# Ledicia/Molecular-Dynamics-Simulation---Lennard-Jones-monoatomic-fluid

Hardware: AMD Instinct MI355X
Metric: md_steps_per_sec_n262144_fp64 (higher is better)
Workload: dtype f64

## Files before the change

molecular-dynamics-simulation---lennard-jones-monoatomic-fluid_amd/csrc/ljmd_common.cpp:

```cpp
#include "ljmd_common.h"
#include "ljmd_internal.h"

#include <algorithm>
#include <cstdio>
#include <cstring>
#include <limits>

namespace ljmdh {

using namespace ljmdk;

thread_local std::string g_last_error = "";

int failv(std::string *handle_err, int code, const char *fmt, va_list ap)
{
    char buf[512];
    vsnprintf(buf, sizeof buf, fmt, ap);
    g_last_error = buf;
    if (handle_err) *handle_err = buf;
    return code;
}

int check_sim_params(const char *who, int n, double box_length, double dt, double rc)
{
// ... 51 lines not shown
        if (v && *v) return std::atoi(v);
        return std::nullopt;
    };
    Knobs k;
    k.sort = flag("LJMD_SORT", k.sort);
    k.force_generic = flag("LJMD_FORCE_GENERIC", k.force_generic);
    k.force_collectives = flag("LJMD_FORCE_COLLECTIVES", k.force_collectives);
    k.fuse = flag("LJMD_FUSE", k.fuse);
    k.fuse_tail = flag("LJMD_FUSE_TAIL", k.fuse_tail);
    k.fuse_defer_record = flag("LJMD_FUSE_DEFER_RECORD", k.fuse_defer_record);
    k.xcd_remap = std::max(0, env_int("LJMD_N3_XCD_REMAP", k.xcd_remap));
    k.inject_failure_at_step = env_int("LJMD_INJECT_FAILURE_AT_STEP", k.inject_failure_at_step);
    k.exchange_alltoall = is("LJMD_FORCE_EXCHANGE", "alltoall");
    k.resort_every = opt_int("LJMD_RESORT_EVERY");
    k.kd_sort_cub = is("LJMD_KD_SORT", "cub");
    k.n3_row_tiles = env_int("LJMD_N3_ROW_TILES", k.n3_row_tiles);
    k.n3_wg_waves = env_int("LJMD_N3_WG_WAVES", k.n3_wg_waves);
    k.slab_budget_gb = std::max(1, env_int("LJMD_SLAB_BUDGET_GB", k.slab_budget_gb));
    k.n3_both_ties = flag("LJMD_N3_BOTH_TIES", k.n3_both_ties);
    k.n3_min_n = env_int("LJMD_N3_MIN_N", k.n3_min_n);
    k.n3 = flag("LJMD_N3", k.n3);
    k.n3_target_waves = opt_int("LJMD_N3_TARGET_WAVES");
    k.n3_clusters = flag("LJMD_N3_CLUSTERS", k.n3_clusters);
    k.n3_pertile = flag("LJMD_N3_PERTILE", k.n3_pertile);
    k.reduce_split = opt_int("LJMD_REDUCE_SPLIT");
    if (k.reduce_split) k.reduce_split = std::max(0, *k.reduce_split);
    k.walk_chunk = opt_int("LJMD_WALK_CHUNK");
    k.vanhove_chunk = opt_int("LJMD_VANHOVE_CHUNK");
    k.fp32_far_stream = flag("LJMD_FP32_FAR_STREAM", k.fp32_far_stream);
    k.fp32_vfar = flag("LJMD_FP32_VFAR", k.fp32_vfar);
    {
        const char *rs = std::getenv("LJMD_FP32_SPLIT");
        if (rs && *rs) k.fp32_split = std::max(0.0, std::atof(rs));
    }
    k.overlap_exchange = flag("LJMD_OVERLAP_EXCHANGE", k.overlap_exchange);
    k.migrate_blocks = is("LJMD_MIGRATE_DEAL", "blocks");
    {
        const char *xm = std::getenv("LJMD_MULTI_EXCHANGE");
        k.multi_exchange = xm ? xm : "";
    }
    k.multi_migrate_every = std::max(0, env_int("LJMD_MULTI_MIGRATE_EVERY", k.multi_migrate_every));
    k.multi_threads = flag("LJMD_MULTI_THREADS", k.multi_threads);
    k.batch_group_streams = !is("LJMD_BATCH_GROUP_STREAMS", "0");
    return k;
}

// ... 72 lines not shown
```

molecular-dynamics-simulation---lennard-jones-monoatomic-fluid_amd/csrc/ljmd_common.h:

```cpp
#ifndef LJMD_COMMON_H
#define LJMD_COMMON_H

#include "ljmd.h"

#include <hip/hip_runtime.h>

#include <cstdarg>
#include <cstddef>
#include <cstdint>
#include <cstdlib>
#include <optional>
#include <string>

namespace ljmdh {

extern thread_local std::string g_last_error;

constexpr double kPi = 3.1415926535897932384626433832795;

int failv(std::string *handle_err, int code, const char *fmt, va_list ap);

inline int fail(std::nullptr_t, int code, const char *fmt, ...)
{
    va_list ap;
// ... 58 lines not shown
void scalars_from_exact_sums(const uint64_t (&ordered)[5][3], double te, double td, double tdd, bool have_e, bool have_k,
                             double *epot, double *ekin, double *d_epot, double *dd_epot);

struct Knobs {
    bool sort = true;
    bool force_generic = false;
    bool force_collectives = false;
    bool fuse = true;
    bool fuse_tail = true;
    bool fuse_defer_record = true;
    int xcd_remap = 4;
    int inject_failure_at_step = -1;
    bool exchange_alltoall = false;
    std::optional<int> resort_every;
    bool kd_sort_cub = false;
    int n3_row_tiles = 0;
    int n3_wg_waves = 0;
    int slab_budget_gb = 64;
    bool n3_both_ties = true;
    int n3_min_n = 4096;
    bool n3 = true;
    std::optional<int> n3_target_waves;
    bool n3_clusters = true;
    bool n3_pertile = true;
    std::optional<int> reduce_split;
    std::optional<int> walk_chunk;
    std::optional<int> vanhove_chunk;
    bool fp32_far_stream = true;
    bool fp32_vfar = true;
    double fp32_split = 5.0;
    bool overlap_exchange = true;
    bool migrate_blocks = false;
    std::string multi_exchange;
    int multi_migrate_every = 2000;
    bool multi_threads = true;
    bool batch_group_streams = true;
};
Knobs read_knobs();

}
#endif
```

molecular-dynamics-simulation---lennard-jones-monoatomic-fluid_amd/csrc/ljmd_engine.cpp:

```cpp
#include "ljmd_engine.h"

namespace ljmdh {

bool fast_path_ok(const ljmd_t *h) { return h->plan.rc_allows_fast && h->positions_compact && !h->knobs.force_generic; }

double *wg_part_now(ljmd_t *h) { return h->d_wg_part + (h->plan.fuse_tail ? (size_t)h->fold_parity * h->wg_part_stride : 0); }

PairArgs pair_args(ljmd_t *h, bool fast)
{
    PairArgs a;
    a.pos = h->d_pos;
    a.slab = h->d_slab;
    a.wg_part = wg_part_now(h);
    a.mask = h->d_mask;
    a.bbox = h->d_bbox;
    a.inline_mask = (fast && h->plan.fuse_tail && !h->plan.use_n3) ? 1 : 0;
    a.rc2_skin = h->rc2 * (1.0 + 1e-10);
    a.n = h->n;
    a.S = h->plan.S;
    a.P = h->plan.P;
    a.G = h->G;
    a.rank = h->rank;
    a.TB = h->plan.TB;
    a.T = h->plan.T;
// ... 42 lines not shown
    a.slab_i = h->d_slab;
    a.slab_j = h->d_slab_j;
    a.flag_j = h->d_flag_j;
    a.wg_part = wg_part_now(h);
    a.S = h->plan.S;
    a.P = h->plan.P;
    a.G = h->G;
    a.rank = h->rank;
    a.TB = h->plan.TB;
    a.T = h->plan.T;
    a.W = h->plan.W;
    a.NG = h->plan.NG;
    a.NGo = h->plan.NGo;
    a.Dmax = h->plan.Dmax;
    a.CS = h->plan.CS;
    a.by_group = h->plan.j_by_group;
    a.dchunk = h->plan.dchunk;
    a.uchunk = h->plan.uchunk;
    a.by0 = 0;
    a.xcd_remap = 0;
    a.inline_class = (h->plan.fuse_tail && h->plan.rt <= 2 && h->plan.wg_waves == 1) ? 1 : 0;
    a.both_ties = h->plan.both_ties ? 1 : 0;
    a.rc2_skin = h->rc2 * (1.0 + 1e-10);
    a.energy = h->want_energy ? 1 : 0;
    a.RT = h->plan.rt;
    a.L = h->L;
    a.invL = h->invL;
    a.rc2 = h->rc2;
    return a;
}

IntegrateArgs integrate_args(ljmd_t *h)
{
    IntegrateArgs a;
    a.r = own_block(h);
    a.ru = h->d_ru;
    a.v = h->d_v;
    a.a = h->d_a;
    a.fsum = needs_force_exchange(h) ? h->d_frecv : h->d_fpart;
    a.bbox = nullptr;
    a.pos_tc = nullptr;
    a.RT = std::max(1, h->plan.rt);
    a.ticket = nullptr;
    a.ke_part = h->d_ke_part;
    a.rows = h->plan.P;
    a.P = h->plan.P;
    a.L = h->L;
// ... 485 lines not shown
```

molecular-dynamics-simulation---lennard-jones-monoatomic-fluid_amd/csrc/ljmd_engine.h:

```cpp
#ifndef LJMD_ENGINE_H
#define LJMD_ENGINE_H

#include "ljmd_common.h"

#include <rccl/rccl.h>

#include <algorithm>
#include <cmath>
#include <cstdio>
#include <cstring>
#include <limits>
#include <mutex>
#include <vector>

#include "ljmd_internal.h"
#include "ljmd_resident.h"
#include "ljmd_sort.h"

using namespace ljmdk;

namespace ljmdh {

constexpr unsigned kRingCap = 4096;
constexpr int kTargetWorkgroups = 2048;
constexpr int kXcdMinGroups = 256;
constexpr int kMixedMinN = 16384;
constexpr long kN3ItemsFor4 = 6000;
constexpr long kN3ItemsFor2 = 1000;
constexpr long kN3LargeItems = 131072;
constexpr int kN3MidTargetItems = 32768;
constexpr int kBothTiesMaxGroups = 128;
constexpr int kFuseTailMaxRowTiles = 2;
constexpr int kFuseTailMaxN = 20000;
constexpr int kReduceSplitMinN = 131072;
constexpr int kReduceSplitShare = 8;
constexpr int kMaxProfiledLaunches = 4096;
constexpr int kEventsPerLaunch = 9;

struct EventSet {
    hipEvent_t e[kEventsPerLaunch];
    bool has_pos_x = false, has_force_x = false;
};

struct LaunchPlan {
    int S = 0, P = 0;
    int TB = 0, T = 0, W = 0;
    bool rc_allows_fast = false;
    bool sort_enabled = true;
    int resort_every = 20;
    std::vector<int> kd_level_nseg;
    std::vector<size_t> kd_level_off;
    std::vector<int> kd_offsets;
    int kd_finish_from = 0;
    int nslab_g = 1, chunk_g = 0;
    int nslab_t = 1, chunk_t = 0;
    bool use_n3 = false;
    int wg_waves = 1;
    bool both_ties = false;
    int uchunk = 0;
    int CS = 0, CS2 = 0, j_by_group = 0;
    int NG = 0, NGo = 0, Dmax = 0, nslab_n = 1, dchunk = 0;
    int rt = kRowTiles;
    bool fuse_tail = false;
    int split_s1 = 0, split_j1 = 0;
    int nslab_max = 1, n_wg_max = 0;
    int n_ke = 0;
};

int plan_engine(const SimParams &sim, int n, int n_ranks, int precision_mode, const Knobs &k, LaunchPlan *out);

}

struct ljmd_multi;

using namespace ljmdh;

struct ljmd : ljmdh::SimParams {
    ljmd_multi *multi = nullptr;
    bool poisoned = false;
    int inject_failure_at = -1;
    int n = 0, rank = 0, G = 1, device = 0, mode = 0;
    ljmdh::Knobs knobs;
// ... 160 lines not shown
```

molecular-dynamics-simulation---lennard-jones-monoatomic-fluid_amd/csrc/ljmd_kernels.hip:

```cpp
#include <hip/hip_runtime.h>
#include <stdint.h>

#include "ljmd_internal.h"

namespace ljmdk {

__device__ __forceinline__ double wave_min(double v)
{
#pragma unroll
    for (int off = 32; off > 0; off >>= 1) v = fmin(v, __shfl_down(v, off, 64));
    return v;
}

__device__ __forceinline__ double wave_max(double v)
{
#pragma unroll
    for (int off = 32; off > 0; off >>= 1) v = fmax(v, __shfl_down(v, off, 64));
    return v;
}

__global__ __launch_bounds__(kBlock) void pair_rows_generic_kernel(PairArgs a)
{
    __shared__ double red[2 * kWavesPerBlock];
    const int row = blockIdx.x * kBlock + threadIdx.x;
// ... 152 lines not shown
}

__device__ __forceinline__ double straddle(double e, double half)
{
    return e - __builtin_copysign(half, e);
}

template <int NU>
__device__ __forceinline__ void pair_disp(double xi, double yi, double zi, double xj, double yj, double zj, double L,
                                          double invL, double sx, double sy, double sz, double &dx, double &dy, double &dz)
{
    static_assert(NU == 7 || NU == 8 || NU == 32 || NU == 33 || NU == 34 || NU == 40, "pair_disp: loop variant");
    dx = xi - xj; dy = yi - yj; dz = zi - zj;
    if constexpr (NU == 7) {
        dx = fma(-L, __builtin_rint(dx * invL), dx);
        dy = fma(-L, __builtin_rint(dy * invL), dy);
        dz = fma(-L, __builtin_rint(dz * invL), dz);
    }
    if constexpr (NU == 32 || NU == 40) dx = straddle(dx, sx);
    if constexpr (NU == 33 || NU == 40) dy = straddle(dy, sy);
    if constexpr (NU == 34 || NU == 40) dz = straddle(dz, sz);
}

template <bool LANE_PRED, int NU, bool INNER = false, bool ENERGY = true>
__device__ __forceinline__ void pair_n3(double xi, double yi, double zi,
                                        double xj, double yj, double zj,
                                        double L, double invL, double rc2, bool lane_ok,
                                        double sx, double sy, double sz,
                                        double &ax, double &ay, double &az,
                                        double &jx, double &jy, double &jz,
                                        double &s12, double &s6)
{
    double dx, dy, dz;
    pair_disp<NU>(xi, yi, zi, xj, yj, zj, L, invL, sx, sy, sz, dx, dy, dz);
    const double r2 = fma(dz, dz, fma(dy, dy, dx * dx));
    bool in = true;
    if constexpr (!INNER) in = r2 < rc2;
    if constexpr (LANE_PRED) in = in && lane_ok;
    if (in) {
        const double u = rcp_newton(r2);
        const double u3 = u * u * u;
        const double u6 = u3 * u3;
        if constexpr (ENERGY) {
            s12 += u6;
            s6 += u3;
        }
        const double g = fma(2.0, u6, -u3) * u;
        ax = fma(g, dx, ax);
        ay = fma(g, dy, ay);
        az = fma(g, dz, az);
        jx = fma(-g, dx, jx);
        jy = fma(-g, dy, jy);
        jz = fma(-g, dz, jz);
    }
}

template <int NU>
__device__ __forceinline__ void pair_geom(double xi, double yi, double zi, double xj, double yj, double zj, double L,
                                          double invL, double sx, double sy, double sz, double &dx, double &dy,
                                          double &dz, double &r2)
{
    pair_disp<NU>(xi, yi, zi, xj, yj, zj, L, invL, sx, sy, sz, dx, dy, dz);
    r2 = fma(dz, dz, fma(dy, dy, dx * dx));
}

template <bool INNER, bool ENERGY>
__device__ __forceinline__ void pair_apply(double u, double dx, double dy, double dz, double r2, double rc2, double &ax,
                                           double &ay, double &az, double &jx, double &jy, double &jz, double &s12,
                                           double &s6)
{
    bool in = true;
    if constexpr (!INNER) in = r2 < rc2;
    if (in) {
        const double u3 = u * u * u;
        const double u6 = u3 * u3;
        if constexpr (ENERGY) {
            s12 += u6;
            s6 += u3;
        }
        const double g = fma(2.0, u6, -u3) * u;
        ax = fma(g, dx, ax);
        ay = fma(g, dy, ay);
        az = fma(g, dz, az);
        jx = fma(-g, dx, jx);
        jy = fma(-g, dy, jy);
        jz = fma(-g, dz, jz);
    }
}

#ifndef LJMD_N3_UNROLL
#define LJMD_N3_UNROLL 8
#endif
#ifndef LJMD_BATCH_RCP
#define LJMD_BATCH_RCP 1
#endif
constexpr int kLdsAxis = 2 * kTile;

template <int RT, int NU, bool MASKED, bool INNER, bool BATCH = false, bool ENERGY = true>
__device__ __forceinline__ void column_tile_loop(const double (&xi)[RT], const double (&yi)[RT],
                                                 const double (&zi)[RT], double (&ax)[RT],
                                                 double (&ay)[RT], double (&az)[RT],
                                                 const double *park, int ns, unsigned mb,
                                                 double L, double invL, double rc2, double sx, double sy, double sz,
                                                 double &jx, double &jy, double &jz, double &s12, double &s6)
{
    static_assert(!BATCH || (!MASKED && (RT == 2 || RT == 4)), "batched reciprocal: all row tiles, 2 or 4 of them");
    static_assert(kTile / 2 % LJMD_N3_UNROLL == 0, "half a pass is a whole number of unrolled bodies");
    double xj, yj, zj;
    double nx = park[kTile], ny = park[kLdsAxis + kTile], nz = park[2 * kLdsAxis + kTile];
    for (int sb = 0; sb < ns; sb += LJMD_N3_UNROLL, park -= LJMD_N3_UNROLL) {
#pragma unroll
    for (int s = 0; s < LJMD_N3_UNROLL; ++s) {
        xj = nx; yj = ny; zj = nz;
        nx = park[kTile - 1 - s];
        ny = park[kLdsAxis + kTile - 1 - s];
        nz = park[2 * kLdsAxis + kTile - 1 - s];
        if constexpr (BATCH) {
            double dx[RT], dy[RT], dz[RT], r2[RT], u[RT];
#pragma unroll
            for (int k = 0; k < RT; ++k)
                pair_geom<NU>(xi[k], yi[k], zi[k], xj, yj, zj, L, invL, sx, sy, sz, dx[k], dy[k], dz[k], r2[k]);
            if constexpr (RT == 4) {
                const double pab = r2[0] * r2[1], pcd = r2[2] * r2[3];
                const double y = rcp_newton(pab * pcd);
                const double rab = y * pcd, rcd = y * pab;
                u[0] = r2[1] * rab; u[1] = r2[0] * rab; u[2] = r2[3] * rcd; u[3] = r2[2] * rcd;
            } else {
                const double y = rcp_newton(r2[0] * r2[1]);
                u[0] = r2[1] * y; u[1] = r2[0] * y;
            }
#pragma unroll
            for (int k = 0; k < RT; ++k)
                pair_apply<INNER, ENERGY>(u[k], dx[k], dy[k], dz[k], r2[k], rc2, ax[k], ay[k], az[k], jx, jy, jz, s12, s6);
        } else {
#pragma unroll
            for (int k = 0; k < RT; ++k)
                if (!MASKED || ((mb >> k) & 1u))
                    pair_n3<false, NU, INNER, ENERGY>(xi[k], yi[k], zi[k], xj, yj, zj, L, invL, rc2, true, sx, sy, sz,
                                              ax[k], ay[k], az[k], jx, jy, jz, s12, s6);
        }
        jx = dpp_rotate(jx); jy = dpp_rotate(jy); jz = dpp_rotate(jz);
    }
    }
}

__device__ __forceinline__ bool uniform_image(double lo, double hi, double L, double invL, double &shift)
{
    const double tlo = lo * invL, thi = hi * invL;
    const double n = __builtin_rint(0.5 * (tlo + thi));
    shift = n * L;
    return (tlo > n - 0.5 + 1e-9) && (thi < n + 0.5 - 1e-9) && (fabs(n) <= 2.0);
}

#ifdef LJMD_VARIANT_STATS
__device__ unsigned long long g_variant_stats[80];
#endif
#ifdef LJMD_WAVE_TRACE
constexpr int kTraceWaves = 1 << 16;
__device__ unsigned long long g_wave_trace[kTraceWaves * 8];
__device__ __forceinline__ unsigned long long trace_now() { return __builtin_amdgcn_s_memrealtime(); }
__device__ __forceinline__ void trace_store(unsigned wave_index, unsigned long long t0, unsigned long long t1, unsigned long long t2,
// ... 198 lines not shown
            const double *pk = parked + 2 * kClu * cl + i;
            const double x0 = pk[kClu], y0 = pk[kLdsAxis + kClu], z0 = pk[2 * kLdsAxis + kClu];
            if (mbc == ((1u << RT) - 1u))
                column_cluster_loop<RT, false, (RT == 2 || RT == 4) && LJMD_BATCH_RCP, ENERGY>(
                    xi, yi, zi, ax, ay, az, x0, y0, z0, pk, mbc, a.rc2, jx, jy, jz, s12, s6);
            else
                column_cluster_loop<RT, true, false, ENERGY>(xi, yi, zi, ax, ay, az, x0, y0, z0, pk, mbc, a.rc2, jx, jy,
                                                             jz, s12, s6);
            jx = rows_sum(jx);
            jy = rows_sum(jy);
            jz = rows_sum(jz);
        }
#ifdef LJMD_VARIANT_STATS
        if (lane == 0) atomicAdd(&g_variant_stats[64 + __builtin_popcount(mbc)], 1ull);
#endif
        if (row == cl) {
            out[slot] = jx;
            out[kTile + slot] = jy;
            out[2 * kTile + slot] = jz;
        }
    }
}

template <int RT, int W, bool ENERGY>
__device__ __forceinline__ void n3_tile_pass(const N3Args &a, int lane, int c, int d, int l, int s0, int ns, unsigned mb,
                                             unsigned desc, const double (&xi)[RT],
                                             const double (&yi)[RT], const double (&zi)[RT], double (&ax)[RT],
                                             double (&ay)[RT], double (&az)[RT], double *parked,
                                             double &jx, double &jy, double &jz, int &s_end, double &s12, double &s6)
{
    const size_t P = a.P;
    const int gj = (a.G == 1) ? 0 : c / a.TB;
    const double *cb = a.pos + (size_t)gj * 3 * P + (size_t)(c - gj * a.TB) * kTile + lane;
    double xj = cb[0], yj = cb[P], zj = cb[2 * P];

    const int nu = (int)((desc >> 4) & 31u);
    const bool inner = ((desc >> 9) & 1u) != 0, full = ((desc >> 10) & 1u) != 0;
    const double sx = (double)((int)((desc >> 11) & 7u) - 2) * a.L;
    const double sy = (double)((int)((desc >> 14) & 7u) - 2) * a.L;
    const double sz = (double)((int)((desc >> 17) & 7u) - 2) * a.L;

    const bool diag = d == 0 && ((mb >> l) & 1u);
    const bool general_all = nu == 7 || diag;
    int loop = 7;
    double hx = 0.0, hy = 0.0, hz = 0.0;
    if (!general_all) {
        xj += sx; yj += sy; zj += sz;
        loop = 8;
        if (nu >= 27 && nu <= 30) {
            const double half = 0.5 * a.L;
            const unsigned st = (desc >> 22) & 7u, sg = (desc >> 25) & 7u;
            if (st & 1u) { hx = half; xj += (sg & 1u) ? half : -half; }
// ... 28 lines not shown
                                      0.0, 0.0, ax[k], ay[k], az[k], jx, jy, jz, s12, s6);
                }
            }
            jx = dpp_rotate(jx); jy = dpp_rotate(jy); jz = dpp_rotate(jz);
        }
        s_end = max(t0, t1);
        return;
    }
    s_end = s0 + ns;
#define LJMD_LOOP(NU_, MASKED_, INNER_)                                                                      \
    column_tile_loop<RT, NU_, MASKED_, INNER_, false, ENERGY>(xi, yi, zi, ax, ay, az, parked + lane - s0, ns, mb, a.L, a.invL,  \
                                                  a.rc2, hx, hy, hz, jx, jy, jz, s12, s6)
#define LJMD_LOOP_ALL(NU_, INNER_)                                                                           \
    column_tile_loop<RT, NU_, false, INNER_, (RT == 2 || RT == 4) && LJMD_BATCH_RCP, ENERGY>(                              \
        xi, yi, zi, ax, ay, az, parked + lane - s0, ns, mb, a.L, a.invL, a.rc2, hx, hy, hz, jx, jy, jz, s12, s6)
    const bool all4 = mb == ((1u << RT) - 1u) && (full || !LJMD_BATCH_RCP);
#ifdef LJMD_VARIANT_STATS
    if (lane == 0)
    {
        atomicAdd(&g_variant_stats[(nu & 31) * 2 + (inner ? 1 : 0)], (unsigned long long)__builtin_popcount(mb));
        atomicAdd(&g_variant_stats[56 + __builtin_popcount(mb)], 1ull);
    }
#endif
    if (loop == 8 && inner) { if (all4) LJMD_LOOP_ALL(8, true); else LJMD_LOOP(8, true, true); }
    else if (loop == 8)     { if (all4) LJMD_LOOP_ALL(8, false); else LJMD_LOOP(8, true, false); }
    else if (loop == 32)    { if (all4) LJMD_LOOP_ALL(32, false); else LJMD_LOOP(32, true, false); }
    else if (loop == 33)    { if (all4) LJMD_LOOP_ALL(33, false); else LJMD_LOOP(33, true, false); }
    else if (loop == 34)    { if (all4) LJMD_LOOP_ALL(34, false); else LJMD_LOOP(34, true, false); }
    else if (loop == 40)    { if (all4) LJMD_LOOP_ALL(40, false); else LJMD_LOOP(40, true, false); }
    else                    { if (all4) LJMD_LOOP_ALL(7, false); else LJMD_LOOP(7, true, false); }
#undef LJMD_LOOP_ALL
#undef LJMD_LOOP
}

template <int RT>
__device__ __forceinline__ bool tile_class(const GeometryArgs &a, double invL, double rc2, int S, int Al, int c,
                                           unsigned &desc_out, unsigned *desc_far, float *desc2)
{
    {
        const int NG = a.T / RT, A = a.rank * (a.TB / RT) + Al, B = c / RT;
        int d = B - A;
        if (d < 0) d += NG;
        if (!(d == 0 || 2 * d < NG || (2 * d == NG && (A < B || a.both_ties)))) return false;
    }
    double glo[3] = {__builtin_inf(), __builtin_inf(), __builtin_inf()};
    double ghi[3] = {-__builtin_inf(), -__builtin_inf(), -__builtin_inf()};
// ... 143 lines not shown
                for (int k = 0; k < RT; ++k) {
                    const double *bb = a.bbox + (size_t)(a.rank * a.TB + RT * Al + k) * kBoxStride;
                    double supp = 0.0;
#pragma unroll
                    for (int q = 0; q < 3; ++q) supp += fmax((double)nf[q] * row_lo(bb, k, q), (double)nf[q] * row_hi(bb, k, q));
                    o[3 + k] = (float)(supp + rc + 1e-3);
                }
                for (int k = RT; k < 4; ++k) o[3 + k] = 0.0f;
                o[7] = 0.0f;
                double colmax = 0.0;
#pragma unroll
                for (int q = 0; q < 3; ++q) colmax += fmax((double)nf[q] * (cbx[q] + sh[q]), (double)nf[q] * (cbx[3 + q] + sh[q]));
                bool useful = false;
                for (int k = 0; k < RT; ++k) useful = useful || (((mb >> k) & 1u) && colmax > (double)o[3 + k]);
                if (useful) cls |= 1u << 20;
            }
        }
    }
    desc_out = mb | cls;
    if (desc_far) desc_far[(size_t)Al * a.T + c] = mb_far | cls | ((unsigned)(vfar && full && mb_far != 0) << 28);
    return true;
}

template <int MIN_WAVES, int RT, int W, bool ENERGY>
__global__ __launch_bounds__(kTile * W, MIN_WAVES) void pair_n3_kernel(N3Args a)
{
    __shared__ double parked_all[W][3 * kLdsAxis];
    __shared__ double comb[W > 1 ? 2 : 1][W][3][W > 1 ? kTile : 1];
    __shared__ int comb_on[2][W];
    const int lane = threadIdx.x & 63;
    const int wv = W == 1 ? 0 : __builtin_amdgcn_readfirstlane((int)(threadIdx.x >> 6));
    unsigned bx = blockIdx.x, by = blockIdx.y;
    if (a.xcd_remap) {
        const unsigned id = blockIdx.y * gridDim.x + blockIdx.x, per = gridDim.x >> 3, C = (unsigned)a.xcd_remap;
        const unsigned xcd = id & 7u, slot = id >> 3, s = slot % per;
        by = slot / per;
        bx = ((s / C) * 8u + xcd) * C + s % C;
    }
    by += (unsigned)a.by0;
#ifdef LJMD_WAVE_TRACE
    const unsigned long long tr0 = trace_now();
    unsigned long long tr1 = tr0;
    unsigned tr_heavy = 0;
#endif
    const int Al = (int)bx * W + wv;
    const bool active = Al < a.NGo;
    const int A = a.rank * a.NGo + Al;
    const int A0 = a.rank * a.NGo + (int)bx * W;
    const size_t P = a.P;
    const double *own = a.pos + (size_t)a.rank * 3 * P;

    double xi[RT], yi[RT], zi[RT];
    double ax[RT], ay[RT], az[RT];
    double s12 = 0.0, s6 = 0.0;
#pragma unroll
    for (int k = 0; k < RT; ++k) {
        const size_t slot = (size_t)(active ? RT * Al + k : 0) * kTile + lane;
        xi[k] = own[slot];
        yi[k] = own[P + slot];
        zi[k] = own[2 * P + slot];
        ax[k] = ay[k] = az[k] = 0.0;
    }

    const int u0 = (int)by * a.uchunk;
    const int nt = max(0, min(a.uchunk, (a.Dmax + W) * RT - u0));
    const bool both = W == 1 && a.both_ties != 0;

    auto tile_of = [&](int t, int &c, int &d, int &l, int &s0, int &ns, size_t &blk, unsigned &desc) -> unsigned {
        const int u = u0 + t;
        const int e = u / RT;
        l = u - e * RT;
        d = e - wv;
        const bool valid = active && d >= 0 && d <= a.Dmax;
        int B = A0 + e;
        if (B >= a.NG) B -= a.NG;
        const bool tie = 2 * d == a.NG;
        const bool work = valid && ((d == 0) || (2 * d < a.NG) || (tie && (A < B || both)));
        c = RT * B + l;
        blk = (size_t)c * a.CS + (size_t)(a.by_group ? (int)bx : e / W);
        s0 = 0;
        ns = kTile;
        if (tie && both) {
            s0 = A < B ? 0 : 1;
            ns = kTile / 2;
// ... 19 lines not shown
            }
            mb = desc & 15u;
            if (d == 0) mb &= (2u << l) - 1u;
        }
        return mb;
    };

    {
        double *parked = parked_all[wv];
        int buf = 0;
        for (int t = 0; t < nt; ++t) {
            int c, d, l, s0, ns;
            size_t blk;
            unsigned desc;
            const unsigned mb = tile_of(t, c, d, l, s0, ns, blk, desc);
            const bool have = mb != 0;
            int s_end = kTile;
#ifdef LJMD_WAVE_TRACE
            if (t == 0) tr1 = trace_now();
            tr_heavy += have ? 1u : 0u;
#endif
            double jx = 0.0, jy = 0.0, jz = 0.0;
            bool stored = false;
            const bool pertile = have && ((desc >> 21) & 1u);
            if (pertile) {
                const int axis = (int)((desc >> 22) & 3u);
#pragma unroll
                for (int k = 0; k < RT; ++k) {
                    const double sh = (double)((int)((desc >> (24 + 2 * k)) & 3u) - 1) * a.L;
                    if (axis == 0) xi[k] -= sh; else if (axis == 1) yi[k] -= sh; else zi[k] -= sh;
                }
            }
            if (have) {
                double p12 = 0.0, p6 = 0.0;
                if constexpr (W == 1 && RT == kRowTiles) {
                    if (((desc >> 20) & 1u) && ns == kTile) {
                        n3_cluster_pass<RT, ENERGY>(a, lane, Al, c, mb, desc, xi, yi, zi, ax, ay, az, parked,
                                                    a.slab_j + blk * (3 * kTile), p12, p6);
                        stored = true;
                    }
                }
                if (!stored)
                    n3_tile_pass<RT, W, ENERGY>(a, lane, c, d, l, s0, ns, mb, desc, xi, yi, zi, ax, ay, az, parked, jx, jy, jz,
                                                s_end, p12, p6);
                s12 += p12;
                s6 += p6;
            }
            if (pertile) {
                const int axis = (int)((desc >> 22) & 3u);
#pragma unroll
                for (int k = 0; k < RT; ++k) {
                    const double x0 = own[(size_t)axis * P + (size_t)(RT * Al + k) * kTile + lane];
                    if (axis == 0) xi[k] = x0; else if (axis == 1) yi[k] = x0; else zi[k] = x0;
                }
            }
            if constexpr (W == 1) {
                if (have && !stored) {
                    double *o = a.slab_j + blk * (3 * kTile) + ((lane - s_end) & (kTile - 1));
                    o[0] = jx;
                    o[kTile] = jy;
                    o[2 * kTile] = jz;
                }
                if (lane == 0) a.flag_j[blk] = have ? 1 : 0;
            } else {
                if (have) {
                    comb[buf][wv][0][lane] = jx;
                    comb[buf][wv][1][lane] = jy;
                    comb[buf][wv][2][lane] = jz;
                }
                if (lane == 0) comb_on[buf][wv] = have ? 1 : 0;
                __syncthreads();
                if (wv == 0) {
                    double tx = 0.0, ty = 0.0, tz = 0.0;
                    bool any = false;
#pragma unroll
                    for (int w = 0; w < W; ++w)
                        if (comb_on[buf][w]) {
// ... 8 lines not shown
                        o[kTile] = ty;
                        o[2 * kTile] = tz;
                    }
                    if (lane == 0) a.flag_j[blk] = any ? 1 : 0;
                }
                buf ^= 1;
            }
        }
    }

#ifdef LJMD_WAVE_TRACE
    const unsigned long long tr2 = trace_now();
#endif
    if (active) {
        double *si = a.slab_i + (size_t)by * 3 * P;
#pragma unroll
        for (int k = 0; k < RT; ++k) {
            const size_t slot = (size_t)(RT * Al + k) * kTile + lane;
            si[slot] = ax[k];
            si[P + slot] = ay[k];
            si[2 * P + slot] = az[k];
        }
    }
    const double t12 = ENERGY ? wave_sum(s12) : __builtin_nan(""), t6 = ENERGY ? wave_sum(s6) : __builtin_nan("");
    if (lane == 0) {
        double *w = a.wg_part + 2 * (((size_t)by * gridDim.x + bx) * W + wv);
        w[0] = t12;
        w[1] = t6;
    }
#ifdef LJMD_WAVE_TRACE
    if (lane == 0) trace_store((unsigned)((blockIdx.y * gridDim.x + blockIdx.x) * W + wv), tr0, tr1, tr2, tr_heavy, blockIdx.y * gridDim.x + blockIdx.x);
#endif
}

__device__ __forceinline__ float dpp_rotate_f32(float v)
{
    const int i = __builtin_amdgcn_update_dpp(__float_as_int(v), __float_as_int(v), 0x13C, 0xF, 0xF, false);
    return __int_as_float(i);
}

template <int GEN, bool ENERGY, bool VFAR = false>
__device__ __forceinline__ void pair_n3_f32(float xi, float yi, float zi, float xj, float yj, float zj,
                                            float Lf, float invLf, float rc2f,
                                            float &ax, float &ay, float &az, float &jx, float &jy, float &jz,
                                            float &s12, float &s6)
{
    float dx = xi - xj, dy = yi - yj, dz = zi - zj;
// ... 941 lines not shown

hipError_t launch_pair_tiles(const PairArgs &a, dim3 grid, hipStream_t s)
{
    hipLaunchKernelGGL(pair_tiles_kernel, grid, dim3(kBlock), 0, s, a);
    return hipGetLastError();
}

hipError_t launch_pair_n3(const N3Args &a, dim3 grid, int wg_waves, hipStream_t s)
{
    if (a.RT == 1 && !a.energy)
        hipLaunchKernelGGL((pair_n3_kernel<3, 1, 1, false>), grid, dim3(kTile), 0, s, a);
    else if (a.RT == 1)
        hipLaunchKernelGGL((pair_n3_kernel<3, 1, 1, true>), grid, dim3(kTile), 0, s, a);
    else if (a.RT == 2 && !a.energy)
        hipLaunchKernelGGL((pair_n3_kernel<3, 2, 1, false>), grid, dim3(kTile), 0, s, a);
    else if (a.RT == 2)
        hipLaunchKernelGGL((pair_n3_kernel<3, 2, 1, true>), grid, dim3(kTile), 0, s, a);
    else if (wg_waves == 4)
        hipLaunchKernelGGL((pair_n3_kernel<3, kRowTiles, 4, true>), grid, dim3(4 * kTile), 0, s, a);
    else if (wg_waves == 2)
        hipLaunchKernelGGL((pair_n3_kernel<3, kRowTiles, 2, true>), grid, dim3(2 * kTile), 0, s, a);
    else if (!a.energy)
        hipLaunchKernelGGL((pair_n3_kernel<3, kRowTiles, 1, false>), grid, dim3(kTile), 0, s, a);
    else
        hipLaunchKernelGGL((pair_n3_kernel<3, kRowTiles, 1, true>), grid, dim3(kTile), 0, s, a);
    return hipGetLastError();
}

hipError_t launch_pair_n3_f32(const N3Args &a, dim3 grid, hipStream_t s)
{
    if (a.energy)
        hipLaunchKernelGGL(pair_n3_f32_kernel<true>, grid, dim3(kTile), 0, s, a);
    else
        hipLaunchKernelGGL(pair_n3_f32_kernel<false>, grid, dim3(kTile), 0, s, a);
    return hipGetLastError();
}

hipError_t launch_tile_boxes(const GeometryArgs &a, hipStream_t s)
{
    hipLaunchKernelGGL(tile_boxes_kernel, dim3((a.T + kWavesPerBlock - 1) / kWavesPerBlock), dim3(kBlock), 0, s, a);
    return hipGetLastError();
}

hipError_t launch_tile_mask(const GeometryArgs &a, hipStream_t s)
{
    hipLaunchKernelGGL(tile_mask_kernel, dim3(a.W, (a.TB + kWavesPerBlock - 1) / kWavesPerBlock), dim3(kBlock), 0, s, a);
// ... 163 lines not shown
```

molecular-dynamics-simulation---lennard-jones-monoatomic-fluid_amd/csrc/ljmd_plan.cpp:

```cpp
#include "ljmd_engine.h"

namespace ljmdh {

namespace {
int rt_align(int uchunk, int rt)
{
    int m = 1;
    while ((m * uchunk) % rt != 0) ++m;
    return m;
}
}

int plan_engine(const SimParams &sim, int n, int n_ranks, int precision_mode, const Knobs &k, LaunchPlan *out)
{
    LaunchPlan p;
    p.S = n / n_ranks;
    p.P = ((p.S + kSlotAlign - 1) / kSlotAlign) * kSlotAlign;
    p.TB = p.P / kTile;
    p.T = n_ranks * p.TB;
    p.W = (p.T + 63) / 64;
    p.rc_allows_fast = sim.rc <= (1.0 - 1e-9) * 0.5 * sim.L;
    p.sort_enabled = k.sort && n >= 1024;
    p.resort_every = std::max(1, k.resort_every.value_or(n >= 1000000 ? 5 : n >= 131072 ? 10 : n > 40000 ? 20
                                                              : n > kFuseTailMaxN ? 50 : 200));
// ... 41 lines not shown
        p.nslab_t = (p.T + p.chunk_t - 1) / p.chunk_t;
    }
    {
        const bool mixed_mode = precision_mode == LJMD_PRECISION_FP32_FORCE;
        int rt = k.n3_row_tiles;
        if (mixed_mode) rt = kRowTiles;
        if (rt != 1 && rt != 2 && rt != kRowTiles) {
            auto items = [&](int cand) { const long ngo = p.TB / cand; return ngo * ((long)n_ranks * ngo / 2 + 1); };
            rt = items(kRowTiles) >= kN3ItemsFor4 ? kRowTiles : items(2) >= kN3ItemsFor2 ? 2 : 1;
        }
        p.rt = rt;
        p.NGo = p.TB / rt;
        p.NG = n_ranks * p.NGo;
        p.Dmax = p.NG / 2;
        int wg = k.n3_wg_waves;
        if (wg != 1 && wg != 2 && wg != 4) {
            const double budget = 1e9 * k.slab_budget_gb;
            const double full = (double)p.T * (n_ranks > 1 ? p.NGo : p.Dmax + 1) * 3.0 * kTile * sizeof(double);
            wg = full <= budget ? 1 : full <= 2.0 * budget ? 2 : 4;
        }
        if (rt != kRowTiles || p.NGo < 16 * wg) wg = 1;
        p.wg_waves = wg;
        p.both_ties = wg == 1 && n_ranks == 1 && !mixed_mode && p.NG <= kBothTiesMaxGroups && k.n3_both_ties;
        p.j_by_group = (n_ranks > 1 || p.NG % wg != 0) ? 1 : 0;
        p.CS = p.j_by_group ? (p.NGo + wg - 1) / wg : (p.Dmax + wg - 1) / wg + 1;
        p.CS2 = n_ranks > 1 ? p.NGo : p.Dmax + 1;
        p.use_n3 = k.n3 && n >= k.n3_min_n && (n_ranks == 1 || p.rc_allows_fast) &&
                   precision_mode != LJMD_PRECISION_FP64_REPRODUCIBLE;
        const int n_off = p.Dmax + p.wg_waves;
        const int n_units = n_off * rt;
        const bool plenty = (long)p.NGo * n_off >= kN3LargeItems || n_ranks > 1;
        const int target_waves = std::max(1, k.n3_target_waves.value_or(plenty ? 131072 : kN3MidTargetItems));
        const int ns_wanted = (target_waves + p.NGo - 1) / p.NGo;
        int ns = std::max(1, std::min(ns_wanted, n_off));
        const bool small_single = n_ranks == 1 && n <= kFuseTailMaxN && rt <= kFuseTailMaxRowTiles;
        const int ns_cap = small_single ? std::max(1, kDirectFoldMax / std::max(1, p.NGo)) : n_units;
        ns = std::min(ns, ns_cap);
        p.dchunk = (n_off + ns - 1) / ns;
        p.uchunk = p.dchunk * rt;
        if (!mixed_mode && ns_wanted > n_off) {
            const int nsu = std::max(1, std::min(std::min(ns_wanted, ns_cap), n_units));
            p.uchunk = (n_units + nsu - 1) / nsu;
        }
        p.nslab_n = (n_units + p.uchunk - 1) / p.uchunk;
    }
    p.fuse_tail = k.fuse && k.fuse_tail && n_ranks == 1 && n <= kFuseTailMaxN && p.rc_allows_fast &&
// ... 26 lines not shown
```

molecular-dynamics-simulation---lennard-jones-monoatomic-fluid_amd/csrc/ljmd_profile.cpp:

```cpp
#include "ljmd_engine.h"
#include "ljmd_multi.h"

extern "C" {

const char *ljmd_pair_kernel_name(const ljmd_t *h)
{
    if (!h) return "";
    if (h->multi) return ljmdm::pair_kernel_name(h);
    if (reproducible(h)) return "pair_fixed_kernel";
    if (!fast_path_ok(h)) return "pair_rows_generic_kernel";
    if (h->plan.use_n3 && h->mode == LJMD_PRECISION_FP32_FORCE) return "pair_n3_f32_kernel";
    return h->plan.use_n3 ? "pair_n3_kernel" : "pair_tiles_kernel";
}

int ljmd_profile_enable(ljmd_t *h, int32_t on)
{
    LJMD_TRY(entry_checks(h, "ljmd_profile_enable", kHandle));
    if (h->multi) return ljmdm::profile_enable(h, on);
    h->profiling = on != 0;
    h->ev_used = 0;
    return LJMD_OK;
}

int ljmd_profile_read(ljmd_t *h, double *ms_avg, int32_t *launches)
{
    return ljmd_profile_read_ex(h, ms_avg, nullptr, launches);
}

namespace {
int profile_read_full(ljmd_t *h, double *ms_avg , double *ms_min , int32_t *launches,
                      double *ms_median = nullptr )
{
    LJMD_HIP(h, hipSetDevice(h->device));
    LJMD_HIP(h, hipStreamSynchronize(h->stream));
    if (h->comm_stream) LJMD_HIP(h, hipStreamSynchronize(h->comm_stream));
// ... 100 lines not shown
```

Before: 57.12.

## Compute LJ energy sums via force-virial identity to skip r^-12 accumulation

Adds a force-sums variant of the Newton-3 pair kernel, on by default for single-rank fp64 runs with n >= 131072. For eligible tile passes it stops accumulating the u^6 (r^-12) term per pair. It instead reconstructs s12 from a virial-style sum of (position - row-group center) dot force, using s12 = 0.5*(virial + s6). The aim is to remove per-pair add work and register pressure, at the cost of extra LDS parking of row forces, bounding-box center computation and a per-tile dot product. Numerical results for the energy change slightly.

```diff
diff --git a/molecular-dynamics-simulation---lennard-jones-monoatomic-fluid_amd/csrc/ljmd_common.cpp b/molecular-dynamics-simulation---lennard-jones-monoatomic-fluid_amd/csrc/ljmd_common.cpp
--- a/molecular-dynamics-simulation---lennard-jones-monoatomic-fluid_amd/csrc/ljmd_common.cpp
+++ b/molecular-dynamics-simulation---lennard-jones-monoatomic-fluid_amd/csrc/ljmd_common.cpp
@@ -97,6 +97,7 @@
     k.n3 = flag("LJMD_N3", k.n3);
     k.n3_target_waves = opt_int("LJMD_N3_TARGET_WAVES");
     k.n3_clusters = flag("LJMD_N3_CLUSTERS", k.n3_clusters);
+    k.n3_force_sums = opt_int("LJMD_N3_FORCE_SUMS");
     k.n3_pertile = flag("LJMD_N3_PERTILE", k.n3_pertile);
     k.reduce_split = opt_int("LJMD_REDUCE_SPLIT");
     if (k.reduce_split) k.reduce_split = std::max(0, *k.reduce_split);
diff --git a/molecular-dynamics-simulation---lennard-jones-monoatomic-fluid_amd/csrc/ljmd_common.h b/molecular-dynamics-simulation---lennard-jones-monoatomic-fluid_amd/csrc/ljmd_common.h
--- a/molecular-dynamics-simulation---lennard-jones-monoatomic-fluid_amd/csrc/ljmd_common.h
+++ b/molecular-dynamics-simulation---lennard-jones-monoatomic-fluid_amd/csrc/ljmd_common.h
@@ -104,6 +104,7 @@
     bool n3 = true;
     std::optional<int> n3_target_waves;
     bool n3_clusters = true;
+    std::optional<int> n3_force_sums;
     bool n3_pertile = true;
     std::optional<int> reduce_split;
     std::optional<int> walk_chunk;
diff --git a/molecular-dynamics-simulation---lennard-jones-monoatomic-fluid_amd/csrc/ljmd_engine.cpp b/molecular-dynamics-simulation---lennard-jones-monoatomic-fluid_amd/csrc/ljmd_engine.cpp
--- a/molecular-dynamics-simulation---lennard-jones-monoatomic-fluid_amd/csrc/ljmd_engine.cpp
+++ b/molecular-dynamics-simulation---lennard-jones-monoatomic-fluid_amd/csrc/ljmd_engine.cpp
@@ -88,7 +88,7 @@
     a.inline_class = (h->plan.fuse_tail && h->plan.rt <= 2 && h->plan.wg_waves == 1) ? 1 : 0;
     a.both_ties = h->plan.both_ties ? 1 : 0;
     a.rc2_skin = h->rc2 * (1.0 + 1e-10);
-    a.energy = h->want_energy ? 1 : 0;
+    a.energy = h->want_energy ? (h->plan.force_sums ? 2 : 1) : 0;
     a.RT = h->plan.rt;
     a.L = h->L;
     a.invL = h->invL;
diff --git a/molecular-dynamics-simulation---lennard-jones-monoatomic-fluid_amd/csrc/ljmd_engine.h b/molecular-dynamics-simulation---lennard-jones-monoatomic-fluid_amd/csrc/ljmd_engine.h
--- a/molecular-dynamics-simulation---lennard-jones-monoatomic-fluid_amd/csrc/ljmd_engine.h
+++ b/molecular-dynamics-simulation---lennard-jones-monoatomic-fluid_amd/csrc/ljmd_engine.h
@@ -33,6 +33,7 @@
 constexpr int kFuseTailMaxRowTiles = 2;
 constexpr int kFuseTailMaxN = 20000;
 constexpr int kReduceSplitMinN = 131072;
+constexpr int kForceSumsMinN = 131072;
 constexpr int kReduceSplitShare = 8;
 constexpr int kMaxProfiledLaunches = 4096;
 constexpr int kEventsPerLaunch = 9;
@@ -58,6 +59,7 @@
     int wg_waves = 1;
     bool both_ties = false;
     int uchunk = 0;
+    bool force_sums = false;
     int CS = 0, CS2 = 0, j_by_group = 0;
     int NG = 0, NGo = 0, Dmax = 0, nslab_n = 1, dchunk = 0;
     int rt = kRowTiles;
diff --git a/molecular-dynamics-simulation---lennard-jones-monoatomic-fluid_amd/csrc/ljmd_kernels.hip b/molecular-dynamics-simulation---lennard-jones-monoatomic-fluid_amd/csrc/ljmd_kernels.hip
--- a/molecular-dynamics-simulation---lennard-jones-monoatomic-fluid_amd/csrc/ljmd_kernels.hip
+++ b/molecular-dynamics-simulation---lennard-jones-monoatomic-fluid_amd/csrc/ljmd_kernels.hip
@@ -198,7 +198,7 @@
     if constexpr (NU == 34 || NU == 40) dz = straddle(dz, sz);
 }
 
-template <bool LANE_PRED, int NU, bool INNER = false, bool ENERGY = true>
+template <bool LANE_PRED, int NU, bool INNER = false, bool ENERGY = true, bool FOLD = false>
 __device__ __forceinline__ void pair_n3(double xi, double yi, double zi,
                                         double xj, double yj, double zj,
                                         double L, double invL, double rc2, bool lane_ok,
@@ -218,7 +218,7 @@
         const double u3 = u * u * u;
         const double u6 = u3 * u3;
         if constexpr (ENERGY) {
-            s12 += u6;
+            if constexpr (!FOLD) s12 += u6;
             s6 += u3;
         }
         const double g = fma(2.0, u6, -u3) * u;
@@ -240,7 +240,7 @@
     r2 = fma(dz, dz, fma(dy, dy, dx * dx));
 }
 
-template <bool INNER, bool ENERGY>
+template <bool INNER, bool ENERGY, bool FOLD = false>
 __device__ __forceinline__ void pair_apply(double u, double dx, double dy, double dz, double r2, double rc2, double &ax,
                                            double &ay, double &az, double &jx, double &jy, double &jz, double &s12,
                                            double &s6)
@@ -251,7 +251,7 @@
         const double u3 = u * u * u;
         const double u6 = u3 * u3;
         if constexpr (ENERGY) {
-            s12 += u6;
+            if constexpr (!FOLD) s12 += u6;
             s6 += u3;
         }
         const double g = fma(2.0, u6, -u3) * u;
@@ -272,7 +272,7 @@
 #endif
 constexpr int kLdsAxis = 2 * kTile;
 
-template <int RT, int NU, bool MASKED, bool INNER, bool BATCH = false, bool ENERGY = true>
+template <int RT, int NU, bool MASKED, bool INNER, bool BATCH = false, bool ENERGY = true, bool FOLD = false>
 __device__ __forceinline__ void column_tile_loop(const double (&xi)[RT], const double (&yi)[RT],
                                                  const double (&zi)[RT], double (&ax)[RT],
                                                  double (&ay)[RT], double (&az)[RT],
@@ -307,12 +307,12 @@
             }
 #pragma unroll
             for (int k = 0; k < RT; ++k)
-                pair_apply<INNER, ENERGY>(u[k], dx[k], dy[k], dz[k], r2[k], rc2, ax[k], ay[k], az[k], jx, jy, jz, s12, s6);
+                pair_apply<INNER, ENERGY, FOLD>(u[k], dx[k], dy[k], dz[k], r2[k], rc2, ax[k], ay[k], az[k], jx, jy, jz, s12, s6);
         } else {
 #pragma unroll
             for (int k = 0; k < RT; ++k)
                 if (!MASKED || ((mb >> k) & 1u))
-                    pair_n3<false, NU, INNER, ENERGY>(xi[k], yi[k], zi[k], xj, yj, zj, L, invL, rc2, true, sx, sy, sz,
+                    pair_n3<false, NU, INNER, ENERGY, FOLD>(xi[k], yi[k], zi[k], xj, yj, zj, L, invL, rc2, true, sx, sy, sz,
                                               ax[k], ay[k], az[k], jx, jy, jz, s12, s6);
         }
         jx = dpp_rotate(jx); jy = dpp_rotate(jy); jz = dpp_rotate(jz);
@@ -557,12 +557,13 @@
     }
 }
 
-template <int RT, int W, bool ENERGY>
+template <int RT, int W, bool ENERGY, bool FSUMS = false>
 __device__ __forceinline__ void n3_tile_pass(const N3Args &a, int lane, int c, int d, int l, int s0, int ns, unsigned mb,
                                              unsigned desc, const double (&xi)[RT],
                                              const double (&yi)[RT], const double (&zi)[RT], double (&ax)[RT],
                                              double (&ay)[RT], double (&az)[RT], double *parked,
-                                             double &jx, double &jy, double &jz, int &s_end, double &s12, double &s6)
+                                             double &jx, double &jy, double &jz, int &s_end, double &s12, double &s6,
+                                             bool fold = false)
 {
     const size_t P = a.P;
     const int gj = (a.G == 1) ? 0 : c / a.TB;
@@ -637,6 +638,17 @@
         atomicAdd(&g_variant_stats[56 + __builtin_popcount(mb)], 1ull);
     }
 #endif
+    if constexpr (FSUMS) {
+        if (fold) {
+#define LJMD_FOLD(MASKED_, INNER_, BATCH_)                                                                        \
+    column_tile_loop<RT, 8, MASKED_, INNER_, BATCH_, ENERGY, true>(xi, yi, zi, ax, ay, az, parked + lane - s0, ns, mb, a.L, \
+                                                                   a.invL, a.rc2, hx, hy, hz, jx, jy, jz, s12, s6)
+            if (inner) { if (all4) LJMD_FOLD(false, true, LJMD_BATCH_RCP != 0); else LJMD_FOLD(true, true, false); }
+            else       { if (all4) LJMD_FOLD(false, false, LJMD_BATCH_RCP != 0); else LJMD_FOLD(true, false, false); }
+#undef LJMD_FOLD
+            return;
+        }
+    }
     if (loop == 8 && inner) { if (all4) LJMD_LOOP_ALL(8, true); else LJMD_LOOP(8, true, true); }
     else if (loop == 8)     { if (all4) LJMD_LOOP_ALL(8, false); else LJMD_LOOP(8, true, false); }
     else if (loop == 32)    { if (all4) LJMD_LOOP_ALL(32, false); else LJMD_LOOP(32, true, false); }
@@ -826,9 +838,22 @@
     return true;
 }
 
-template <int MIN_WAVES, int RT, int W, bool ENERGY>
+__device__ __forceinline__ double *row_sums_park()
+{
+    __shared__ double park[3 * kRowTiles * kTile];
+    return park;
+}
+__device__ __forceinline__ double wave_uniform(double v)
+{
+    int hi = __double2hiint(v), lo = __double2loint(v);
+    asm volatile("" : "+v"(hi), "+v"(lo));
+    return __hiloint2double(__builtin_amdgcn_readfirstlane(hi), __builtin_amdgcn_readfirstlane(lo));
+}
+
+template <int MIN_WAVES, int RT, int W, bool ENERGY, bool FSUMS = false>
 __global__ __launch_bounds__(kTile * W, MIN_WAVES) void pair_n3_kernel(N3Args a)
 {
+    static_assert(!FSUMS || (ENERGY && W == 1 && RT == kRowTiles), "force-sum energies: one wave, 4-tile row groups");
     __shared__ double parked_all[W][3 * kLdsAxis];
     __shared__ double comb[W > 1 ? 2 : 1][W][3][W > 1 ? kTile : 1];
     __shared__ int comb_on[2][W];
@@ -864,6 +889,29 @@
         yi[k] = own[P + slot];
         zi[k] = own[2 * P + slot];
         ax[k] = ay[k] = az[k] = 0.0;
+    }
+    double wsum = 0.0, ccx = 0.0, ccy = 0.0, ccz = 0.0;
+    bool rows_full = false;
+    if constexpr (FSUMS) {
+        rows_full = active && (RT * Al + RT) * kTile <= a.S;
+        {
+            const int Ab = active ? Al : 0;
+            double lo[3], hi[3];
+#pragma unroll
+            for (int q = 0; q < 3; ++q) {
+                lo[q] = __builtin_inf();
+                hi[q] = -__builtin_inf();
+#pragma unroll
+                for (int k = 0; k < RT; ++k) {
+                    const double *bb = a.bbox + (size_t)(a.rank * a.TB + RT * Ab + k) * kBoxStride;
+                    lo[q] = fmin(lo[q], bb[q]);
+                    hi[q] = fmax(hi[q], bb[3 + q]);
+                }
+            }
+            ccx = wave_uniform(0.5 * (lo[0] + hi[0]));
+            ccy = wave_uniform(0.5 * (lo[1] + hi[1]));
+            ccz = wave_uniform(0.5 * (lo[2] + hi[2]));
+        }
     }
 
     const int u0 = (int)by * a.uchunk;
@@ -929,6 +977,8 @@
 #endif
             double jx = 0.0, jy = 0.0, jz = 0.0;
             bool stored = false;
+            double fs_pw = 0.0;
+            bool fs_unfold = false;
             const bool pertile = have && ((desc >> 21) & 1u);
             if (pertile) {
                 const int axis = (int)((desc >> 22) & 3u);
@@ -940,6 +990,36 @@
             }
             if (have) {
                 double p12 = 0.0, p6 = 0.0;
+                if constexpr (FSUMS) {
+                    const unsigned nu = (desc >> 4) & 31u;
+                    const bool cluster = ((desc >> 20) & 1u) && ns == kTile;
+                    const bool fold = rows_full && ((desc >> 10) & 1u) && !pertile && d != 0 && nu != 7u && !(nu >= 27u && nu <= 30u) &&
+                                      !cluster;
+                    double *rp = row_sums_park() + lane;
+                    if (!fold && rows_full) {
+#pragma unroll
+                        for (int k = 0; k < RT; ++k) {
+                            rp[(3 * k) * kTile] = ax[k];
+                            rp[(3 * k + 1) * kTile] = ay[k];
+                            rp[(3 * k + 2) * kTile] = az[k];
+                        }
+                    }
+                    if (cluster) {
+                        n3_cluster_pass<RT, ENERGY>(a, lane, Al, c, mb, desc, xi, yi, zi, ax, ay, az, parked,
+                                                    a.slab_j + blk * (3 * kTile), p12, p6);
+                        stored = true;
+                    } else {
+                        n3_tile_pass<RT, W, ENERGY, true>(a, lane, c, d, l, s0, ns, mb, desc, xi, yi, zi, ax, ay, az, parked,
+                                                          jx, jy, jz, s_end, p12, p6, fold);
+                        if (fold) {
+                            const double *pj = parked + ((lane - s_end) & (kTile - 1));
+                            p12 = fma(pj[2 * kLdsAxis] - ccz, jz, fma(pj[kLdsAxis] - ccy, jy, (pj[0] - ccx) * jx));
+                        }
+                    }
+                    fs_pw = fold ? p12 : fma(2.0, p12, -p6);
+                    fs_unfold = !fold && rows_full;
+                    s6 += p6;
+                } else {
                 if constexpr (W == 1 && RT == kRowTiles) {
                     if (((desc >> 20) & 1u) && ns == kTile) {
                         n3_cluster_pass<RT, ENERGY>(a, lane, Al, c, mb, desc, xi, yi, zi, ax, ay, az, parked,
@@ -952,6 +1032,7 @@
                                                 s_end, p12, p6);
                 s12 += p12;
                 s6 += p6;
+                }
             }
             if (pertile) {
                 const int axis = (int)((desc >> 22) & 3u);
@@ -960,6 +1041,20 @@
                     const double x0 = own[(size_t)axis * P + (size_t)(RT * Al + k) * kTile + lane];
                     if (axis == 0) xi[k] = x0; else if (axis == 1) yi[k] = x0; else zi[k] = x0;
                 }
+            }
+            if constexpr (FSUMS) {
+                if (fs_unfold) {
+                    const double *rp = row_sums_park() + lane;
+                    double rterm = 0.0;
+#pragma unroll
+                    for (int k = 0; k < RT; ++k) {
+                        rterm = fma(xi[k] - ccx, ax[k] - rp[(3 * k) * kTile], rterm);
+                        rterm = fma(yi[k] - ccy, ay[k] - rp[(3 * k + 1) * kTile], rterm);
+                        rterm = fma(zi[k] - ccz, az[k] - rp[(3 * k + 2) * kTile], rterm);
+                    }
+                    fs_pw -= rterm;
+                }
+                wsum += fs_pw;
             }
             if constexpr (W == 1) {
                 if (have && !stored) {
@@ -1014,7 +1109,16 @@
             si[2 * P + slot] = az[k];
         }
     }
-    const double t12 = ENERGY ? wave_sum(s12) : __builtin_nan(""), t6 = ENERGY ? wave_sum(s6) : __builtin_nan("");
+    double t12 = ENERGY ? wave_sum(s12) : __builtin_nan("");
+    const double t6 = ENERGY ? wave_sum(s6) : __builtin_nan("");
+    if constexpr (FSUMS) {
+        if (rows_full) {
+#pragma unroll
+            for (int k = 0; k < RT; ++k)
+                wsum = fma(zi[k] - ccz, az[k], fma(yi[k] - ccy, ay[k], fma(xi[k] - ccx, ax[k], wsum)));
+        }
+        t12 = 0.5 * (wave_sum(wsum) + t6);
+    }
     if (lane == 0) {
         double *w = a.wg_part + 2 * (((size_t)by * gridDim.x + bx) * W + wv);
         w[0] = t12;
@@ -2002,6 +2106,8 @@
         hipLaunchKernelGGL((pair_n3_kernel<3, kRowTiles, 2, true>), grid, dim3(2 * kTile), 0, s, a);
     else if (!a.energy)
         hipLaunchKernelGGL((pair_n3_kernel<3, kRowTiles, 1, false>), grid, dim3(kTile), 0, s, a);
+    else if (a.energy == 2)
+        hipLaunchKernelGGL((pair_n3_kernel<3, kRowTiles, 1, true, true>), grid, dim3(kTile), 0, s, a);
     else
         hipLaunchKernelGGL((pair_n3_kernel<3, kRowTiles, 1, true>), grid, dim3(kTile), 0, s, a);
     return hipGetLastError();
diff --git a/molecular-dynamics-simulation---lennard-jones-monoatomic-fluid_amd/csrc/ljmd_plan.cpp b/molecular-dynamics-simulation---lennard-jones-monoatomic-fluid_amd/csrc/ljmd_plan.cpp
--- a/molecular-dynamics-simulation---lennard-jones-monoatomic-fluid_amd/csrc/ljmd_plan.cpp
+++ b/molecular-dynamics-simulation---lennard-jones-monoatomic-fluid_amd/csrc/ljmd_plan.cpp
@@ -87,6 +87,8 @@
         if (rt != kRowTiles || p.NGo < 16 * wg) wg = 1;
         p.wg_waves = wg;
         p.both_ties = wg == 1 && n_ranks == 1 && !mixed_mode && p.NG <= kBothTiesMaxGroups && k.n3_both_ties;
+        p.force_sums = n_ranks == 1 && precision_mode == LJMD_PRECISION_FP64 && rt == kRowTiles && wg == 1 &&
+                       k.n3_force_sums.value_or(n >= kForceSumsMinN ? 1 : 0) != 0;
         p.j_by_group = (n_ranks > 1 || p.NG % wg != 0) ? 1 : 0;
         p.CS = p.j_by_group ? (p.NGo + wg - 1) / wg : (p.Dmax + wg - 1) / wg + 1;
         p.CS2 = n_ranks > 1 ? p.NGo : p.Dmax + 1;
diff --git a/molecular-dynamics-simulation---lennard-jones-monoatomic-fluid_amd/csrc/ljmd_profile.cpp b/molecular-dynamics-simulation---lennard-jones-monoatomic-fluid_amd/csrc/ljmd_profile.cpp
--- a/molecular-dynamics-simulation---lennard-jones-monoatomic-fluid_amd/csrc/ljmd_profile.cpp
+++ b/molecular-dynamics-simulation---lennard-jones-monoatomic-fluid_amd/csrc/ljmd_profile.cpp
@@ -11,6 +11,23 @@
     if (!fast_path_ok(h)) return "pair_rows_generic_kernel";
     if (h->plan.use_n3 && h->mode == LJMD_PRECISION_FP32_FORCE) return "pair_n3_f32_kernel";
     return h->plan.use_n3 ? "pair_n3_kernel" : "pair_tiles_kernel";
+}
+
+int ljmd_debug_pass_descriptors(ljmd_t *h, uint32_t *out, int64_t cap, int32_t *rows, int32_t *cols, int32_t *force_sums)
+{
+    LJMD_TRY(entry_checks(h, "ljmd_debug_pass_descriptors", kHandle));
+    if (h->multi || !h->plan.use_n3 || !h->d_desc)
+        return fail(h, LJMD_ERR_STATE, "ljmd_debug_pass_descriptors: one engine with the Newton-3 kernel's descriptors");
+    const int64_t cnt = (int64_t)h->plan.NGo * h->plan.T;
+    if (rows) *rows = h->plan.NGo;
+    if (cols) *cols = h->plan.T;
+    if (force_sums) *force_sums = h->plan.force_sums ? 1 : 0;
+    if (!out) return LJMD_OK;
+    if (cap < cnt) return fail(h, LJMD_ERR_INVALID_ARG, "ljmd_debug_pass_descriptors: %lld words needed", (long long)cnt);
+    LJMD_HIP(h, hipSetDevice(h->device));
+    LJMD_HIP(h, hipStreamSynchronize(h->stream));
+    LJMD_HIP(h, hipMemcpy(out, h->d_desc, (size_t)cnt * sizeof(uint32_t), hipMemcpyDeviceToHost));
+    return LJMD_OK;
 }
 
 int ljmd_profile_enable(ljmd_t *h, int32_t on)
```

After: 57.34, median of 3. Within noise of the previous version (+0.4%).
